# alexcoca/DistributedKernelShap

Hardware: AMD Instinct MI355X
Metric: explanations/sec (2560 inst, 100-sample background) (higher is better)
Workload: dtype fp32; 1 GPU; model=adult-logreg (12 groups, D=50, n_out=2, logit link), global_batch=2560, background=100, nsamples=default(2M+2048), parallelism=dp1, device=cuda

## Files before the change

distributedkernelshap_amd/ops/hip/bindings.cpp:

```cpp
#include <torch/extension.h>
#include <ATen/hip/HIPContext.h>
#include <c10/hip/HIPStream.h>

#include <cstdint>

extern "C" void launch_fill_random_masks(
    uint8_t* masks, int B, int S, int M, int ne, int n_random,
    const float* cdf, const int* sizes, int n_sizes, int num_paired,
    uint32_t seed, const int32_t* inst_ids, hipStream_t stream);

extern "C" int launch_fused_predict_linear(
    const uint8_t* masksU, const float* diff, const float* base, const float* wbg,
    float* ey, int B, int S, int M, int Mpad, int Npad, int n_out, int act,
    hipStream_t stream);

extern "C" void launch_synth_chunk(
    const uint8_t* masks, const float* x, const float* bg, const int* col_group,
    void* out, int out_bf16, int S, int M, int N, int D, int b_lo, int b_hi,
    int s_lo, int s_hi, hipStream_t stream);

extern "C" void launch_pack_masks(
    const uint8_t* masks, uint64_t* packed, int B, int S, int M,
    hipStream_t stream);

extern "C" int launch_fused_predict_bf16(
    const uint8_t* masksU, const uint16_t* diffB,
    const float* base, const float* wbg, float* ey, int B, int S, int M,
    int Npad, int n_out, int act, int split, hipStream_t stream);

extern "C" void launch_build_diff_f32(
    const float* xp, const float* bgp, const int64_t* vidx, float* out,
    int B, int G, int O, int N, int m, int Mpad, int Npad, hipStream_t stream);

extern "C" void launch_build_diff_bf16(
    const float* xp, const float* bgp, const int64_t* vidx, uint16_t* out,
    int B, int G, int O, int N, int m, int Npad, int split, hipStream_t stream);

extern "C" int launch_wls_solve(
    const uint8_t* masks, const uint64_t* packed, const float* kw,
    const float* ey_adj, const float* total, float* phi, int B, int S, int M,
    int n_out, hipStream_t stream);

extern "C" void launch_pack_masks_words(
    const uint8_t* masks, uint64_t* packed, int B, int S, int M, int W,
    hipStream_t stream);

extern "C" int launch_wls_gram(
    const uint64_t* packed, const float* kw, const float* ey_adj,
    const float* total, double* A64, double* rhs64, int B, int S, int M,
    int W, int n_out, hipStream_t stream);

extern "C" int launch_fused_predict_tiled(
    const uint8_t* masksU, const float* diff, const float* base,
    const float* wbg, float* partial, float* ey, int B, int S, int M,
    int Mpad, int Npad, int n_out, int act, hipStream_t stream);

extern "C" void launch_build_diff_bf16_tiled(
    const float* xp, const float* bgp, const int64_t* vidx, uint16_t* out,
    int B, int G, int O, int N, int m, int Mpad, int Npad, int split,
    hipStream_t stream);

extern "C" int launch_fused_predict_tiled_bf16(
    const uint8_t* masksU, const uint16_t* diffB, const float* base,
    const float* wbg, float* partial, float* ey, int B, int S, int M,
    int Mpad, int Npad, int n_out, int act, int split, hipStream_t stream);

extern "C" int launch_fill_masks_packed(
    uint64_t* packed, const uint64_t* enum_packed, int B, int S, int M, int ne,
    int n_random, const float* cdf, const int* sizes, int n_sizes,
    int num_paired, uint32_t seed, const int32_t* inst_ids, hipStream_t stream);

extern "C" int launch_linear_prepare(
    const float* X, const float* W, const float* bias,
    const int64_t* col_group, const int64_t* vidx, const float* bgp,
    const double* lfnull64, float* diff, float* total, int B, int D, int G,
    int N, int m, int Mpad, int Npad, int n_out, int act, int link,
    hipStream_t stream);

extern "C" int launch_fused_predict_linear_packed(
    const uint64_t* packed, const float* diff, const float* base,
    const float* wbg, const float* lfnull, float* ey, int B, int S, int Mpad,
    int Npad, int n_out, int act, int link, hipStream_t stream, int mma);

extern "C" int launch_wls_solve_packed(
    const uint64_t* packed, const float* kw, const float* ey_adj,
    const float* total, const int64_t* vidx, float* phi_full, int B, int S,
    int M, int n_out, int G, hipStream_t stream);

extern "C" int launch_varying_probe(
    const float* X, const float* bg_min, const float* bg_max,
    const float* tol_min, const float* tol_max, const int64_t* col_group,
    int64_t* keys, int64_t* probe, int B, int D, int G, hipStream_t stream);

extern "C" int launch_fused_predict_mlp(
    const uint8_t* masks, const void* xp1, const void* bgp1n,
    const float* base1, const void* const* hw, const float* const* hb,
    const int* H, int nhid, const void* wout, const float* bout,
    const float* wbg, float* ey, int B, int S, int M, int Mpad, int N,
    int n_out, int act, int hidden_act, int is_bf16, int nsplit,
    hipStream_t stream);

extern "C" int launch_fused_predict_trees(
    const uint8_t* masks, const int* vmap, const int64_t* dx, const int64_t* dbg,
    const uint8_t* child, const int* meta, const float* leaves,
    const int* grp_off, const int* grp_id, const int64_t* grp_mask,
    const float* base, const float* wbg, float* ey, float scale,
    int B, int S, int Mv, int N, int T, int G, int E, int L, int C,
    int max_internal, int n_out, int act, int leaf_mode, hipStream_t stream);

extern "C" int launch_fused_predict_trees_walk(
    const uint8_t* masks, const int* vmap, const float* x, const float* bg,
    const int* nodes, const int* roots, const float* leaves, const float* base,
    const float* wbg, float* ey, float scale,
    int B, int S, int Mv, int N, int D, int G, int T, int R, int L,
    int max_depth, int n_out, int act, int leaf_mode,
    const unsigned* cat_left, int C, hipStream_t stream);

extern "C" int launch_fused_predict_kernelmachine(
    const uint8_t* masks, const float* xp, const float* bgpn,
    const float* base, const float* alpha, const float* icpt,
    const float* wbg, float* ey, int B, int S, int M, int Mpad, int N,
    int Vpad, int n_out, int act, int kernel, float gamma, float coef0,
    int degree, hipStream_t stream);

namespace {

#define CHECK_DEV(t) TORCH_CHECK((t).is_cuda() && (t).is_contiguous(), #t " must be a contiguous device tensor")

hipStream_t current_stream() {
    return c10::hip::getCurrentHIPStream().stream();
}

void fill_random_masks(
    torch::Tensor masks, int64_t ne, int64_t n_random,
    torch::Tensor cdf, torch::Tensor sizes, int64_t num_paired, int64_t seed,
    torch::Tensor inst_ids) {
    CHECK_DEV(masks); CHECK_DEV(cdf); CHECK_DEV(sizes); CHECK_DEV(inst_ids);
    TORCH_CHECK(masks.dtype() == torch::kUInt8, "masks must be uint8");
    TORCH_CHECK(masks.dim() == 3, "masks must be (B,S,M)");
    TORCH_CHECK(inst_ids.dtype() == torch::kInt32, "inst_ids must be int32");
    int B = masks.size(0), S = masks.size(1), M = masks.size(2);
    TORCH_CHECK(inst_ids.size(0) == B, "inst_ids length");
    TORCH_CHECK(M <= 256, "fill_random_masks supports M <= 256");
    launch_fill_random_masks(
        masks.data_ptr<uint8_t>(), B, S, M, (int)ne, (int)n_random,
        cdf.data_ptr<float>(), sizes.data_ptr<int>(), (int)cdf.size(0),
        (int)num_paired, (uint32_t)seed, inst_ids.data_ptr<int32_t>(),
        current_stream());
}

void fused_predict_linear(
    torch::Tensor masks, torch::Tensor diff, torch::Tensor base,
    torch::Tensor wbg, torch::Tensor ey, int64_t act) {
    CHECK_DEV(masks); CHECK_DEV(diff); CHECK_DEV(base); CHECK_DEV(wbg); CHECK_DEV(ey);
    TORCH_CHECK(masks.dtype() == torch::kUInt8, "masks must be u8 (B,S,M)");
    int B = masks.size(0), S = masks.size(1), M = masks.size(2);
    int Mpad = diff.size(2), Npad = diff.size(3);
    int n_out = ey.size(2);
    int oimg = (act == 3) ? 1 : n_out;
    TORCH_CHECK(diff.size(1) == oimg, "diff image count vs act");
    TORCH_CHECK(M <= Mpad, "M vs Mpad");
    TORCH_CHECK(ey.size(0) == B && ey.size(1) == S, "ey shape");
    TORCH_CHECK(base.size(0) == oimg && base.size(1) == Npad, "base shape");
    TORCH_CHECK(wbg.size(0) == Npad, "wbg shape");
    int rc = launch_fused_predict_linear(
        masks.data_ptr<uint8_t>(), diff.data_ptr<float>(), base.data_ptr<float>(),
        wbg.data_ptr<float>(), ey.data_ptr<float>(), B, S, M, Mpad, Npad,
        n_out, (int)act, current_stream());
    TORCH_CHECK(rc == 0, "fused_predict_linear: unsupported shape (Mpad<=64, Npad%16==0, Npad<=128, n_out in {1,2,4})");
}

void synth_chunk(
    torch::Tensor masks, torch::Tensor x, torch::Tensor bg,
    torch::Tensor col_group, torch::Tensor out, int64_t b_lo, int64_t b_hi,
    int64_t s_lo, int64_t s_hi) {
    CHECK_DEV(masks); CHECK_DEV(x); CHECK_DEV(bg); CHECK_DEV(col_group); CHECK_DEV(out);
    int S = masks.size(1), M = masks.size(2);
    int N = bg.size(0), D = bg.size(1);
    TORCH_CHECK(out.size(0) == (b_hi - b_lo) * (s_hi - s_lo) * N && out.size(1) == D,
                "out shape");
    const bool bf16 = out.dtype() == torch::kBFloat16;
    TORCH_CHECK(bf16 || out.dtype() == torch::kFloat32,
                "out must be float32 or bfloat16");
    launch_synth_chunk(
        masks.data_ptr<uint8_t>(), x.data_ptr<float>(), bg.data_ptr<float>(),
        col_group.data_ptr<int>(),
        bf16 ? (void*)out.data_ptr<at::BFloat16>()
             : (void*)out.data_ptr<float>(),
        bf16 ? 1 : 0, S, M, N, D,
        (int)b_lo, (int)b_hi, (int)s_lo, (int)s_hi, current_stream());
}

void wls_solve(
    torch::Tensor masks, torch::Tensor kw, torch::Tensor ey_adj,
    torch::Tensor total, torch::Tensor phi,
    c10::optional<torch::Tensor> packed) {
    CHECK_DEV(masks); CHECK_DEV(kw); CHECK_DEV(ey_adj); CHECK_DEV(total); CHECK_DEV(phi);
    int B = masks.size(0), S = masks.size(1), M = masks.size(2);
    int n_out = ey_adj.size(2);
    TORCH_CHECK(phi.size(0) == B && phi.size(1) == M && phi.size(2) == n_out, "phi shape");
    const uint64_t* pk = nullptr;
    if (packed.has_value()) {
        CHECK_DEV(packed.value());
        TORCH_CHECK(packed->size(0) == B && packed->size(1) == S, "packed shape");
        pk = reinterpret_cast<const uint64_t*>(packed->data_ptr<int64_t>());
    }
    int rc = launch_wls_solve(
        masks.data_ptr<uint8_t>(), pk, kw.data_ptr<float>(), ey_adj.data_ptr<float>(),
        total.data_ptr<float>(), phi.data_ptr<float>(), B, S, M, n_out,
        current_stream());
    TORCH_CHECK(rc == 0, "wls_solve: unsupported shape (2<=M<=64, n_out<=8)");
}

void pack_masks(torch::Tensor masks, torch::Tensor packed) {
    CHECK_DEV(masks); CHECK_DEV(packed);
    TORCH_CHECK(masks.dtype() == torch::kUInt8, "masks must be u8");
    int B = masks.size(0), S = masks.size(1), M = masks.size(2);
    TORCH_CHECK(M <= 64, "pack_masks supports M <= 64");
    TORCH_CHECK(packed.size(0) == B && packed.size(1) == S, "packed shape");
    launch_pack_masks(
        masks.data_ptr<uint8_t>(),
        reinterpret_cast<uint64_t*>(packed.data_ptr<int64_t>()),
        B, S, M, current_stream());
}

#define CHECK_F32(t) TORCH_CHECK((t).dtype() == torch::kFloat32, #t " must be float32")
#define CHECK_I64(t) TORCH_CHECK((t).dtype() == torch::kInt64, #t " must be int64")

void fill_masks_packed(
    torch::Tensor packed, torch::Tensor enum_packed, int64_t n_random,
    torch::Tensor cdf, torch::Tensor sizes, int64_t num_paired, int64_t seed,
    torch::Tensor inst_ids, int64_t M) {
    CHECK_DEV(packed); CHECK_DEV(enum_packed); CHECK_DEV(cdf); CHECK_DEV(sizes);
    CHECK_DEV(inst_ids);
    CHECK_I64(packed); CHECK_I64(enum_packed); CHECK_F32(cdf);
    TORCH_CHECK(sizes.dtype() == torch::kInt32, "sizes must be int32");
    TORCH_CHECK(inst_ids.dtype() == torch::kInt32, "inst_ids must be int32");
    TORCH_CHECK(packed.dim() == 2 && enum_packed.dim() == 1,
                "packed must be (B,S), enum_packed (ne,)");
    int B = packed.size(0), S = packed.size(1), ne = enum_packed.size(0);
    TORCH_CHECK(inst_ids.dim() == 1 && inst_ids.size(0) == B, "inst_ids length");
    TORCH_CHECK(n_random >= 0 && ne + n_random == S, "ne + n_random must equal S");
    TORCH_CHECK(cdf.dim() == 1 && sizes.dim() == 1
                && cdf.size(0) == sizes.size(0), "cdf vs sizes");
    TORCH_CHECK(n_random == 0 || cdf.size(0) >= 1, "empty size table");
    int rc = launch_fill_masks_packed(
        reinterpret_cast<uint64_t*>(packed.data_ptr<int64_t>()),
        reinterpret_cast<const uint64_t*>(enum_packed.data_ptr<int64_t>()),
        B, S, (int)M, ne, (int)n_random, cdf.data_ptr<float>(),
        sizes.data_ptr<int>(), (int)cdf.size(0), (int)num_paired,
        (uint32_t)seed, inst_ids.data_ptr<int32_t>(), current_stream());
    TORCH_CHECK(rc == 0, "fill_masks_packed: unsupported shape (1<=M<=64)");
}

void linear_prepare(
    torch::Tensor X, torch::Tensor W, torch::Tensor bias,
    torch::Tensor col_group, torch::Tensor vidx, torch::Tensor bgp,
    torch::Tensor lfnull64, torch::Tensor diff, torch::Tensor total,
    int64_t act, int64_t link) {
    CHECK_DEV(X); CHECK_DEV(W); CHECK_DEV(bias); CHECK_DEV(col_group);
    CHECK_DEV(vidx); CHECK_DEV(bgp); CHECK_DEV(lfnull64); CHECK_DEV(diff);
    CHECK_DEV(total);
    CHECK_F32(X); CHECK_F32(W); CHECK_F32(bias); CHECK_F32(bgp); CHECK_F32(diff);
    CHECK_F32(total); CHECK_I64(col_group); CHECK_I64(vidx);
    TORCH_CHECK(lfnull64.dtype() == torch::kFloat64, "lfnull64 must be float64");
    TORCH_CHECK(X.dim() == 2 && W.dim() == 2 && bgp.dim() == 3 && diff.dim() == 4
                && total.dim() == 2 && vidx.dim() == 1, "operand ranks");
    int B = X.size(0), D = X.size(1), n_out = W.size(0);
    int N = bgp.size(0), G = bgp.size(1), OI = bgp.size(2), m = vidx.size(0);
    int Mpad = diff.size(2), Npad = diff.size(3);
    TORCH_CHECK(W.size(1) == D && bias.numel() == n_out
                && col_group.numel() == D && lfnull64.numel() == n_out,
                "W (n_out,D), b (n_out), col_group (D), lfnull64 (n_out)");
    TORCH_CHECK(OI == (act == 3 ? 1 : n_out), "background image count vs act");
    TORCH_CHECK(diff.size(0) == B && diff.size(1) == OI, "diff (B,OI,Mpad,Npad)");
    TORCH_CHECK(total.size(0) == B && total.size(1) == n_out, "total (B,n_out)");
    TORCH_CHECK(link == 0 || link == 1, "link must be 0 or 1");
    int rc = launch_linear_prepare(
        X.data_ptr<float>(), W.data_ptr<float>(), bias.data_ptr<float>(),
        col_group.data_ptr<int64_t>(), vidx.data_ptr<int64_t>(),
        bgp.data_ptr<float>(), lfnull64.data_ptr<double>(),
        diff.data_ptr<float>(), total.data_ptr<float>(), B, D, G, N, m, Mpad,
        Npad, n_out, (int)act, (int)link, current_stream());
    TORCH_CHECK(rc == 0, "linear_prepare: unsupported shape (m<=Mpad, m<=64, "
                         "N<=Npad, n_out<=8, act 3 needs n_out==2)");
}

void fused_predict_linear_packed(
    torch::Tensor packed, torch::Tensor diff, torch::Tensor base,
    torch::Tensor wbg, torch::Tensor ey, int64_t act, int64_t link,
    c10::optional<torch::Tensor> lfnull, int64_t mma) {
    CHECK_DEV(packed); CHECK_DEV(diff); CHECK_DEV(base); CHECK_DEV(wbg); CHECK_DEV(ey);
    CHECK_I64(packed); CHECK_F32(diff); CHECK_F32(base); CHECK_F32(wbg); CHECK_F32(ey);
    TORCH_CHECK(packed.dim() == 2 && diff.dim() == 4 && ey.dim() == 3
                && base.dim() == 2, "operand ranks");
    int B = packed.size(0), S = packed.size(1);
    int Mpad = diff.size(2), Npad = diff.size(3);
    int n_out = ey.size(2);
    int oimg = (act == 3) ? 1 : n_out;
    TORCH_CHECK(diff.size(0) == B && diff.size(1) == oimg, "diff (B,oimg,Mpad,Npad) vs act");
    TORCH_CHECK(ey.size(0) == B && ey.size(1) == S, "ey shape");
    TORCH_CHECK(base.size(0) == oimg && base.size(1) == Npad, "base shape");
    TORCH_CHECK(wbg.numel() == Npad, "wbg shape");
    const float* lf = nullptr;
    if (lfnull.has_value()) {
        CHECK_DEV(lfnull.value()); CHECK_F32(lfnull.value());
        TORCH_CHECK(lfnull->numel() == n_out, "lfnull must be (n_out,)");
        lf = lfnull->data_ptr<float>();
    }
    TORCH_CHECK(link == 0 || (link == 1 && lf != nullptr),
                "link must be 0, or 1 with lfnull given");
    TORCH_CHECK(mma >= -1 && mma <= 1,
                "mma must be -1 (auto), 0 (fp32 MFMA) or 1 (split bf16 MFMA)");
    int rc = launch_fused_predict_linear_packed(
        reinterpret_cast<const uint64_t*>(packed.data_ptr<int64_t>()),
        diff.data_ptr<float>(), base.data_ptr<float>(), wbg.data_ptr<float>(),
        lf, ey.data_ptr<float>(), B, S, Mpad, Npad, n_out, (int)act, (int)link,
        current_stream(), (int)mma);
    TORCH_CHECK(rc == 0, "fused_predict_linear_packed: unsupported shape "
                         "(Mpad%4==0, Mpad<=64, Npad%16==0, Npad<=128, n_out in "
                         "{1,2,4}, operand images within 64 KiB of LDS)");
}

void wls_solve_packed(
    torch::Tensor packed, torch::Tensor kw, torch::Tensor ey_adj,
    torch::Tensor total, torch::Tensor vidx, torch::Tensor phi_full) {
    CHECK_DEV(packed); CHECK_DEV(kw); CHECK_DEV(ey_adj); CHECK_DEV(total);
    CHECK_DEV(vidx); CHECK_DEV(phi_full);
    CHECK_I64(packed); CHECK_F32(kw); CHECK_F32(ey_adj); CHECK_F32(total);
    CHECK_I64(vidx); CHECK_F32(phi_full);
    TORCH_CHECK(packed.dim() == 2 && ey_adj.dim() == 3 && phi_full.dim() == 3
                && vidx.dim() == 1 && total.dim() == 2, "operand ranks");
    int B = packed.size(0), S = packed.size(1), M = vidx.size(0);
    int n_out = ey_adj.size(2), G = phi_full.size(1);
    TORCH_CHECK(kw.numel() == S, "kw must be (S,)");
    TORCH_CHECK(ey_adj.size(0) == B && ey_adj.size(1) == S, "ey_adj shape");
    TORCH_CHECK(total.size(0) == B && total.size(1) == n_out, "total shape");
    TORCH_CHECK(phi_full.size(0) == B && phi_full.size(2) == n_out, "phi_full shape");
    int rc = launch_wls_solve_packed(
        reinterpret_cast<const uint64_t*>(packed.data_ptr<int64_t>()),
        kw.data_ptr<float>(), ey_adj.data_ptr<float>(), total.data_ptr<float>(),
        vidx.data_ptr<int64_t>(), phi_full.data_ptr<float>(), B, S, M, n_out,
        G, current_stream());
    TORCH_CHECK(rc == 0, "wls_solve_packed: unsupported shape (2<=M<=G, "
                         "(M-1)+n_out<=16)");
}

void varying_probe(
    torch::Tensor X, torch::Tensor bg_min, torch::Tensor bg_max,
    torch::Tensor tol_min, torch::Tensor tol_max, torch::Tensor col_group,
    int64_t n_groups, torch::Tensor keys, torch::Tensor probe) {
    CHECK_DEV(X); CHECK_DEV(bg_min); CHECK_DEV(bg_max); CHECK_DEV(tol_min);
    CHECK_DEV(tol_max); CHECK_DEV(col_group); CHECK_DEV(keys); CHECK_DEV(probe);
    CHECK_F32(X); CHECK_F32(bg_min); CHECK_F32(bg_max); CHECK_F32(tol_min);
    CHECK_F32(tol_max); CHECK_I64(col_group); CHECK_I64(keys); CHECK_I64(probe);
    TORCH_CHECK(X.dim() == 2, "X must be (B,D)");
    const int64_t B = X.size(0), D = X.size(1);
    TORCH_CHECK(B >= 1 && D >= 1 && B <= 0x7fffffffLL && D <= 0x7fffffffLL,
                "X must be (B,D) with B, D >= 1");
    TORCH_CHECK(bg_min.numel() == D && bg_max.numel() == D
                && tol_min.numel() == D && tol_max.numel() == D
                && col_group.numel() == D,
                "bg_min, bg_max, tol_min, tol_max, col_group must be (D,)");
    TORCH_CHECK(keys.numel() == B, "keys must be (B,)");
    TORCH_CHECK(probe.numel() == 2, "probe must be (2,)");
    int rc = launch_varying_probe(
        X.data_ptr<float>(), bg_min.data_ptr<float>(), bg_max.data_ptr<float>(),
        tol_min.data_ptr<float>(), tol_max.data_ptr<float>(),
        col_group.data_ptr<int64_t>(), keys.data_ptr<int64_t>(),
        probe.data_ptr<int64_t>(), (int)B, (int)D, (int)n_groups,
        current_stream());
    TORCH_CHECK(rc == 0, "varying_probe: unsupported shape (1 <= n_groups <= 62)");
}

void fused_predict_bf16(
    torch::Tensor masks, torch::Tensor diffB, torch::Tensor base,
    torch::Tensor wbg, torch::Tensor ey, int64_t act) {
    CHECK_DEV(masks); CHECK_DEV(diffB); CHECK_DEV(base); CHECK_DEV(wbg); CHECK_DEV(ey);
    TORCH_CHECK(masks.dtype() == torch::kUInt8 && diffB.dtype() == torch::kBFloat16);
    int B = masks.size(0), S = masks.size(1), M = masks.size(2);
    int split = diffB.size(1), Npad = diffB.size(3);
    int n_out = ey.size(2);
    TORCH_CHECK(diffB.size(2) == ((act == 3) ? 1 : n_out), "diffB image count vs act");
    TORCH_CHECK(diffB.size(0) == B && diffB.size(4) == 40, "diffB (B,split,o,Npad,40)");
    TORCH_CHECK(ey.size(0) == B && ey.size(1) == S, "ey shape");
    int rc = launch_fused_predict_bf16(
        masks.data_ptr<uint8_t>(),
        reinterpret_cast<const uint16_t*>(diffB.data_ptr<at::BFloat16>()),
        base.data_ptr<float>(), wbg.data_ptr<float>(), ey.data_ptr<float>(),
        B, S, M, Npad, n_out, (int)act, split, current_stream());
    TORCH_CHECK(rc == 0, "fused_predict_bf16: unsupported shape (M<=32, Npad<=128, n_out in {1,2,4}, split in {1,2})");
}

void build_diff_f32(torch::Tensor xp, torch::Tensor bgp, torch::Tensor vidx,
                    torch::Tensor out) {
    CHECK_DEV(xp); CHECK_DEV(bgp); CHECK_DEV(vidx); CHECK_DEV(out);
    int B = xp.size(0), G = xp.size(1), O = xp.size(2);
    int N = bgp.size(0), m = vidx.size(0);
    int Mpad = out.size(2), Npad = out.size(3);
    TORCH_CHECK(out.size(0) == B && out.size(1) == O && m <= Mpad && N <= Npad);
    launch_build_diff_f32(
        xp.data_ptr<float>(), bgp.data_ptr<float>(), vidx.data_ptr<int64_t>(),
        out.data_ptr<float>(), B, G, O, N, m, Mpad, Npad, current_stream());
}

void build_diff_bf16(torch::Tensor xp, torch::Tensor bgp, torch::Tensor vidx,
                     torch::Tensor out) {
    CHECK_DEV(xp); CHECK_DEV(bgp); CHECK_DEV(vidx); CHECK_DEV(out);
    TORCH_CHECK(out.dtype() == torch::kBFloat16 && out.size(4) == 40);
    int B = xp.size(0), G = xp.size(1), O = xp.size(2);
    int N = bgp.size(0), m = vidx.size(0);
    int split = out.size(1), Npad = out.size(3);
    TORCH_CHECK(out.size(0) == B && out.size(2) == O && N <= Npad && m <= 32);
    launch_build_diff_bf16(
        xp.data_ptr<float>(), bgp.data_ptr<float>(), vidx.data_ptr<int64_t>(),
        reinterpret_cast<uint16_t*>(out.data_ptr<at::BFloat16>()), B, G, O, N,
        m, Npad, split, current_stream());
}

void pack_masks_words(torch::Tensor masks, torch::Tensor packed) {
    CHECK_DEV(masks); CHECK_DEV(packed);
    TORCH_CHECK(masks.dtype() == torch::kUInt8, "masks must be u8");
    TORCH_CHECK(packed.dim() == 3, "packed must be (B,S,W)");
    int B = masks.size(0), S = masks.size(1), M = masks.size(2);
    int W = packed.size(2);
    TORCH_CHECK(packed.size(0) == B && packed.size(1) == S, "packed shape");
    TORCH_CHECK(W * 64 >= M, "packed word count vs M");
    launch_pack_masks_words(
        masks.data_ptr<uint8_t>(),
        reinterpret_cast<uint64_t*>(packed.data_ptr<int64_t>()),
        B, S, M, W, current_stream());
}

void wls_gram(
    torch::Tensor packed, torch::Tensor kw, torch::Tensor ey_adj,
    torch::Tensor total, torch::Tensor A64, torch::Tensor rhs64) {
    CHECK_DEV(packed); CHECK_DEV(kw); CHECK_DEV(ey_adj); CHECK_DEV(total);
    CHECK_DEV(A64); CHECK_DEV(rhs64);
    TORCH_CHECK(packed.dim() == 3, "packed must be (B,S,W)");
    TORCH_CHECK(A64.dtype() == torch::kFloat64 && rhs64.dtype() == torch::kFloat64);
    int B = packed.size(0), S = packed.size(1), W = packed.size(2);
    int mm = A64.size(1), n_out = ey_adj.size(2);
    TORCH_CHECK(A64.size(0) == B && A64.size(2) == mm, "A64 shape");
    TORCH_CHECK(rhs64.size(0) == B && rhs64.size(1) == mm
                && rhs64.size(2) == n_out, "rhs64 shape");
    TORCH_CHECK(W * 64 >= mm + 1, "packed word count vs M");
    int rc = launch_wls_gram(
        reinterpret_cast<const uint64_t*>(packed.data_ptr<int64_t>()),
        kw.data_ptr<float>(), ey_adj.data_ptr<float>(),
        total.data_ptr<float>(), A64.data_ptr<double>(),
        rhs64.data_ptr<double>(), B, S, mm + 1, W, n_out, current_stream());
    TORCH_CHECK(rc == 0, "wls_gram: unsupported shape (M<=513, n_out<=8)");
}

void fused_predict_tiled(
    torch::Tensor masks, torch::Tensor diff, torch::Tensor base,
    torch::Tensor wbg, torch::Tensor partial, torch::Tensor ey, int64_t act) {
    CHECK_DEV(masks); CHECK_DEV(diff); CHECK_DEV(base); CHECK_DEV(wbg);
    CHECK_DEV(partial); CHECK_DEV(ey);
    TORCH_CHECK(masks.dtype() == torch::kUInt8, "masks must be u8 (B,S,M)");
    int B = masks.size(0), S = masks.size(1), M = masks.size(2);
    int Mpad = diff.size(2), Npad = diff.size(3);
    int n_out = ey.size(2);
    int oimg = (act == 3) ? 1 : n_out;
    int nacc = n_out;
    int n_ntiles = (Npad + 127) / 128;
    TORCH_CHECK(diff.size(1) == oimg, "diff image count vs act");
    TORCH_CHECK(M <= Mpad, "M vs Mpad");
    TORCH_CHECK(ey.size(0) == B && ey.size(1) == S, "ey shape");
    TORCH_CHECK(base.size(0) == oimg && base.size(1) == Npad, "base shape");
    TORCH_CHECK(wbg.size(0) == Npad, "wbg shape");
    TORCH_CHECK(partial.size(0) == B && partial.size(1) == n_ntiles
                && partial.size(2) == S && partial.size(3) == nacc,
                "partial shape (B, n_ntiles, S, nacc)");
    int rc = launch_fused_predict_tiled(
        masks.data_ptr<uint8_t>(), diff.data_ptr<float>(),
        base.data_ptr<float>(), wbg.data_ptr<float>(),
        partial.data_ptr<float>(), ey.data_ptr<float>(), B, S, M, Mpad,
        Npad, n_out, (int)act, current_stream());
    TORCH_CHECK(rc == 0, "fused_predict_tiled: unsupported shape "
                         "(Mpad%16==0, Npad%16==0, n_out in {1,2,4})");
}

void build_diff_bf16_tiled(torch::Tensor xp, torch::Tensor bgp,
                           torch::Tensor vidx, torch::Tensor out) {
    CHECK_DEV(xp); CHECK_DEV(bgp); CHECK_DEV(vidx); CHECK_DEV(out);
    TORCH_CHECK(out.dtype() == torch::kBFloat16 && out.dim() == 5,
                "out must be bf16 (B,split,O,Npad,Mpad)");
    int B = xp.size(0), G = xp.size(1), O = xp.size(2);
    int N = bgp.size(0), mcount = vidx.size(0);
    int split = out.size(1), Npad = out.size(3), Mpad = out.size(4);
    TORCH_CHECK(out.size(0) == B && out.size(2) == O && N <= Npad
                && mcount <= Mpad);
    launch_build_diff_bf16_tiled(
        xp.data_ptr<float>(), bgp.data_ptr<float>(), vidx.data_ptr<int64_t>(),
        reinterpret_cast<uint16_t*>(out.data_ptr<at::BFloat16>()), B, G, O, N,
        mcount, Mpad, Npad, split, current_stream());
}
// ... 186 lines not shown
    const int N = bg.size(0);
    TORCH_CHECK(nodes.dtype() == torch::kInt32 && nodes.dim() == 2
                && nodes.size(1) == 4, "nodes must be int32 (R,4)");
    TORCH_CHECK(roots.dtype() == torch::kInt32 && roots.dim() == 1,
                "roots must be int32 (T)");
    TORCH_CHECK(leaf_mode == 0 || leaf_mode == 1, "leaf_mode must be 0 or 1");
    TORCH_CHECK(leaves.dtype() == torch::kFloat32
                && (leaf_mode == 0 ? leaves.dim() == 1
                                   : (leaves.dim() == 2 && leaves.size(1) == n_out)),
                "leaves must be f32 (L) for scalar or (L,n_out) for vector leaves");
    TORCH_CHECK(base.dtype() == torch::kFloat32 && base.numel() == n_out,
                "base must be f32 (n_out)");
    TORCH_CHECK(wbg.dtype() == torch::kFloat32 && wbg.numel() == N,
                "wbg must be f32 (N)");
    TORCH_CHECK(max_depth >= 0 && max_depth <= 64, envelope);
    const unsigned* cat_ptr = nullptr;
    int64_t C = 0;
    if (cat_left.has_value()) {
        const torch::Tensor& cl = *cat_left;
        CHECK_DEV(cl);
        TORCH_CHECK(cl.dtype() == torch::kInt32 && cl.dim() == 2
                    && cl.size(1) == 8 && cl.size(0) >= 1,
                    "cat_left must be int32 (C,8) with C >= 1");
        TORCH_CHECK(cl.size(0) <= 0x7fffffffLL / 8, envelope);
        cat_ptr = reinterpret_cast<const unsigned*>(cl.data_ptr<int>());
        C = cl.size(0);
    }
    TORCH_CHECK(nodes.size(0) <= 0x7fffffffLL && leaves.size(0) <= 0x7fffffffLL
                && roots.size(0) <= 0x7fffffffLL && D <= 0x7fffffffLL
                && vmap.size(0) <= 0x7fffffffLL, envelope);
    int rc = launch_fused_predict_trees_walk(
        masks.data_ptr<uint8_t>(), vmap.data_ptr<int>(), x.data_ptr<float>(),
        bg.data_ptr<float>(), nodes.data_ptr<int>(), roots.data_ptr<int>(),
        leaves.data_ptr<float>(), base.data_ptr<float>(), wbg.data_ptr<float>(),
        ey.data_ptr<float>(), (float)scale, B, S, Mv, N, (int)D,
        (int)vmap.size(0), (int)roots.size(0), (int)nodes.size(0),
        (int)leaves.size(0), (int)max_depth, n_out, (int)act, (int)leaf_mode,
        cat_ptr, (int)C, current_stream());
    TORCH_CHECK(rc != -2, "fused_predict_trees_walk: LDS size attribute rejected");
    TORCH_CHECK(rc == 0, envelope);
}

void fused_predict_kernelmachine(
    torch::Tensor masks, torch::Tensor xp, torch::Tensor bgpn,
    torch::Tensor base, torch::Tensor alpha, torch::Tensor intercept,
    torch::Tensor wbg, torch::Tensor ey, int64_t kernel, double gamma,
    double coef0, int64_t degree, int64_t act) {
    static const char* envelope =
        "fused_predict_kernelmachine: outside the supported envelope (rbf or "
        "poly of degree 1-8, at most 2048 support vectors after padding to "
        "16, n_out <= 8, M <= Mpad <= 64 with Mpad a multiple of 16)";
    CHECK_DEV(masks); CHECK_DEV(xp); CHECK_DEV(bgpn); CHECK_DEV(base);
    CHECK_DEV(alpha); CHECK_DEV(intercept); CHECK_DEV(wbg); CHECK_DEV(ey);
    TORCH_CHECK(masks.dtype() == torch::kUInt8 && masks.dim() == 3,
                "masks must be u8 (B,S,M)");
    TORCH_CHECK(xp.dtype() == torch::kFloat32 && xp.dim() == 3,
                "xp must be f32 (B,Vpad,Mpad)");
    const int B = masks.size(0), S = masks.size(1), M = masks.size(2);
    const int Vpad = xp.size(1), Mpad = xp.size(2);
    TORCH_CHECK(xp.size(0) == B, "xp must be f32 (B,Vpad,Mpad)");
    TORCH_CHECK(bgpn.dtype() == torch::kFloat32 && bgpn.dim() == 3
                && bgpn.size(1) == Vpad && bgpn.size(2) == Mpad,
                "bgpn must be f32 (N,Vpad,Mpad)");
    const int N = bgpn.size(0);
    TORCH_CHECK(base.dtype() == torch::kFloat32 && base.dim() == 2
                && base.size(0) == N && base.size(1) == Vpad,
                "base must be f32 (N,Vpad)");
    TORCH_CHECK(alpha.dtype() == torch::kFloat32 && alpha.dim() == 2
                && alpha.size(0) == 16 && alpha.size(1) == Vpad,
                "alpha must be f32 (16,Vpad)");
    TORCH_CHECK(intercept.dtype() == torch::kFloat32 && intercept.numel() == 16,
                "intercept must be f32 (16)");
    TORCH_CHECK(wbg.dtype() == torch::kFloat32 && wbg.numel() == N,
                "wbg must be f32 (N)");
    TORCH_CHECK(ey.dtype() == torch::kFloat32 && ey.dim() == 3
                && ey.size(0) == B && ey.size(1) == S,
                "ey must be f32 (B,S,n_out)");
    const int n_out = ey.size(2);
    int rc = launch_fused_predict_kernelmachine(
        masks.data_ptr<uint8_t>(), xp.data_ptr<float>(), bgpn.data_ptr<float>(),
        base.data_ptr<float>(), alpha.data_ptr<float>(),
        intercept.data_ptr<float>(), wbg.data_ptr<float>(),
        ey.data_ptr<float>(), B, S, M, Mpad, N, Vpad, n_out, (int)act,
        (int)kernel, (float)gamma, (float)coef0, (int)degree, current_stream());
    TORCH_CHECK(rc == 0, envelope);
}

}

PYBIND11_MODULE(TORCH_EXTENSION_NAME, m) {
    m.def("fused_predict_kernelmachine", &fused_predict_kernelmachine,
          "fused kernel-machine predict (K4k): distance / dot product folded "
          "over varying groups, support vectors streamed in tiles of 16, "
          "kernel evaluation and the contraction with alpha on chip",
          pybind11::arg("masks"), pybind11::arg("xp"), pybind11::arg("bgpn"),
          pybind11::arg("base"), pybind11::arg("alpha"),
          pybind11::arg("intercept"), pybind11::arg("wbg"), pybind11::arg("ey"),
          pybind11::arg("kernel"), pybind11::arg("gamma"),
          pybind11::arg("coef0"), pybind11::arg("degree"), pybind11::arg("act"));
    m.def("fused_predict_trees", &fused_predict_trees,
          "fused tree-ensemble predict (K4t): per-tree node masks in LDS, "
          "bitwise select of packed x / background decisions, bit-register walk",
          pybind11::arg("masks"), pybind11::arg("vmap"), pybind11::arg("dx"),
          pybind11::arg("dbg"), pybind11::arg("child"), pybind11::arg("meta"),
          pybind11::arg("leaves"), pybind11::arg("grp_off"),
          pybind11::arg("grp_id"), pybind11::arg("grp_mask"),
          pybind11::arg("base"), pybind11::arg("scale"), pybind11::arg("wbg"),
          pybind11::arg("ey"), pybind11::arg("act"), pybind11::arg("leaf_mode"),
          pybind11::arg("max_internal"));
    m.def("fused_predict_trees_walk", &fused_predict_trees_walk,
          "fused deep-tree predict (K4w): 16-byte node records walked on the "
          "blended row, group bitset per sample, x row and background in LDS",
          pybind11::arg("masks"), pybind11::arg("vmap"), pybind11::arg("x"),
          pybind11::arg("bg"), pybind11::arg("nodes"), pybind11::arg("roots"),
          pybind11::arg("leaves"), pybind11::arg("base"),
          pybind11::arg("scale"), pybind11::arg("wbg"), pybind11::arg("ey"),
          pybind11::arg("act"), pybind11::arg("leaf_mode"),
          pybind11::arg("max_depth"),
          pybind11::arg("cat_left") = pybind11::none());
    m.def("fused_predict_mlp", &fused_predict_mlp,
          "fused MLP predict (K4m): first layer folded over varying groups, "
          "hidden activations in LDS, f32 or bf16 MFMA by operand dtype",
          pybind11::arg("masks"), pybind11::arg("xp1"), pybind11::arg("bgp1n"),
          pybind11::arg("base1"), pybind11::arg("hidden_w"),
          pybind11::arg("hidden_b"), pybind11::arg("wout"),
          pybind11::arg("bout"), pybind11::arg("wbg"), pybind11::arg("ey"),
          pybind11::arg("act"), pybind11::arg("hidden_act") = 0);
    m.def("fill_masks_packed", &fill_masks_packed,
          "Philox coalition sampling straight into packed u64 words (K2p): "
          "bit-identical to the enumerated-row copy, fill_random_masks and "
          "pack_masks in sequence, M <= 64",
          pybind11::arg("packed"), pybind11::arg("enum_packed"),
          pybind11::arg("n_random"), pybind11::arg("cdf"),
          pybind11::arg("sizes"), pybind11::arg("num_paired"),
          pybind11::arg("seed"), pybind11::arg("inst_ids"), pybind11::arg("M"));
    m.def("linear_prepare", &linear_prepare,
          "per-call operand prep for the packed linear pipeline (K0p): diff "
          "image in the build_diff_f32 layout plus the fp64-evaluated totals",
          pybind11::arg("X"), pybind11::arg("W"), pybind11::arg("b"),
          pybind11::arg("col_group"), pybind11::arg("vidx"),
          pybind11::arg("bgp"), pybind11::arg("lfnull64"),
          pybind11::arg("diff"), pybind11::arg("total"), pybind11::arg("act"),
          pybind11::arg("link"));
    m.def("fused_predict_linear_packed", &fused_predict_linear_packed,
          "MFMA fused predict from packed mask words with the link fused into "
          "the epilogue (K3p); mma: -1 auto, 0 fp32 MFMA, 1 split-operand bf16 "
          "MFMA (Mpad <= 12, act 1/3; other shapes take the fp32 MFMA path)",
          pybind11::arg("packed"), pybind11::arg("diff"), pybind11::arg("base"),
          pybind11::arg("wbg"), pybind11::arg("ey"), pybind11::arg("act"),
          pybind11::arg("link") = 0, pybind11::arg("lfnull") = pybind11::none(),
          pybind11::arg("mma") = -1);
    m.def("wls_solve_packed", &wls_solve_packed,
          "MFMA WLS solve with (S,) kernel weights, scattered into "
          "phi_full (B,G,n_out) through vidx (K7p)",
          pybind11::arg("packed"), pybind11::arg("kw"), pybind11::arg("ey_adj"),
          pybind11::arg("total"), pybind11::arg("vidx"),
          pybind11::arg("phi_full"));
    m.def("varying_probe", &varying_probe,
          "varying-pattern probe (K1p): per-instance group bit keys and "
          "[all(keys == keys[0]), keys[0]] in two launches, no host sync",
          pybind11::arg("X"), pybind11::arg("bg_min"), pybind11::arg("bg_max"),
          pybind11::arg("tol_min"), pybind11::arg("tol_max"),
          pybind11::arg("col_group"), pybind11::arg("n_groups"),
          pybind11::arg("keys"), pybind11::arg("probe"));
    m.def("fill_random_masks", &fill_random_masks,
          "Philox coalition sampling (K2)");
    m.def("fused_predict_linear", &fused_predict_linear,
          "MFMA fused mask@diff GEMM + activation + background reduce (K3-K6)");
    m.def("build_diff_f32", &build_diff_f32,
          "diff image in the f32 fused-kernel layout");
    m.def("build_diff_bf16", &build_diff_bf16,
          "hi(+lo) diff images in the bf16 fused-kernel layout");
    m.def("pack_masks", &pack_masks,
          "masks u8 -> packed u64 bits (for the MFMA WLS Gram build)");
    m.def("fused_predict_bf16", &fused_predict_bf16,
          "bf16 matrix-core fused predict (single or hi+lo split), A-operand "
          "converted in-register from the raw u8 masks");
    m.def("synth_chunk", &synth_chunk,
          "masked-background perturbation synthesis tile (K3')");
    m.def("wls_solve", &wls_solve,
          "batched constrained WLS Shapley solve (K7)",
          pybind11::arg("masks"), pybind11::arg("kw"), pybind11::arg("ey_adj"),
          pybind11::arg("total"), pybind11::arg("phi"),
          pybind11::arg("packed") = pybind11::none());
    m.def("pack_masks_words", &pack_masks_words,
          "masks u8 -> (B,S,W) packed u64 words (wide-M Gram build)");
    m.def("wls_gram", &wls_gram,
          "tiled MFMA Gram+rhs build (fp64 via chunked promotion) for the "
          "stress WLS shapes, M up to 513");
    m.def("fused_predict_tiled", &fused_predict_tiled,
          "tiled MFMA fused predict for Mpad>64 / Npad>128 (LDS-streamed "
          "diff chunks, per-column-tile partials + deterministic reduce)");
    m.def("build_diff_bf16_tiled", &build_diff_bf16_tiled,
          "hi(+lo) k-contiguous diff image for the bf16 tiled predict");
    m.def("fused_predict_tiled_bf16", &fused_predict_tiled_bf16,
          "bf16 matrix-core tiled fused predict (v_mfma_f32_16x16x32_bf16 "
          "per 32-deep k block; hi+lo split for fp32-grade)");
}
```

distributedkernelshap_amd/ops/hip/kshap_kernels.hip:

```cpp

#include <hip/hip_runtime.h>
#include <cstdint>
#include <type_traits>

#include "split_bf16.h"

#define WAVE 64


struct Philox {
    uint32_t ctr[4];
    uint32_t key[2];
    uint32_t buf[4];
    int idx;

    __device__ void init(uint32_t k0, uint32_t k1, uint32_t c0, uint32_t c1) {
        key[0] = k0; key[1] = k1;
        ctr[0] = c0; ctr[1] = c1; ctr[2] = 0; ctr[3] = 0;
        idx = 4;
    }
    __device__ static void round_(uint32_t c[4], const uint32_t k[2]) {
        const uint32_t M0 = 0xD2511F53u, M1 = 0xCD9E8D57u;
        uint64_t p0 = (uint64_t)M0 * c[0];
        uint64_t p1 = (uint64_t)M1 * c[2];
// ... 2355 lines not shown
                           : arow == 2 ? partial[o][2] : partial[o][3];
            }
            if (link == 1) {
#pragma unroll
                for (int o = 0; o < NOUT; ++o) {
                    const float p = fminf(fmaxf(out[o], 1e-7f), 0.9999999f);
                    out[o] = 0.69314718055994530942f
                        * (__builtin_amdgcn_logf(p) - __builtin_amdgcn_logf(1.0f - p));
                }
            }
            if (lfnull != nullptr) {
#pragma unroll
                for (int o = 0; o < NOUT; ++o) out[o] -= lfnull[o];
            }
            float* dst = ey + ((size_t)b * S + ss) * NOUT;
            if constexpr (NOUT == 2) {
                *(float2*)dst = make_float2(out[0], out[1]);
            } else if constexpr (NOUT == 4) {
                *(float4*)dst = make_float4(out[0], out[1], out[2], out[3]);
            } else {
                dst[0] = out[0];
            }
        }
    }
}

template <int NOUT, int ACT, int NT>
static int launch_fpp_ks(
    const uint64_t* packed, const float* diff, const float* base,
    const float* wbg, const float* lfnull, float* ey, int B, int S, int Mpad,
    int link, int mma, hipStream_t stream)
{
    const int n_stiles = (S + S_TILE - 1) / S_TILE;
    dim3 grid(B * n_stiles), block(256);
    constexpr int NPAD = NT * 16;
    constexpr int NSTRIDE = NPAD + ((16 - (NPAD & 31)) & 31);
    constexpr int OIMG = (ACT == 3) ? 1 : NOUT;
    size_t lds = (size_t)(OIMG * Mpad * NSTRIDE + OIMG * NPAD + NPAD) * 4;
    if (lds > 64 * 1024) return -1;
#define KSHAP_FPP(KSV, MMAV) \
    fused_predict_linear_packed_kernel<NOUT, ACT, NT, KSV, MMAV> \
        <<<grid, block, lds, stream>>>(packed, diff, base, wbg, lfnull, ey, \
                                       B, S, Mpad, link)
    if constexpr (ACT == 1 || ACT == 3) {
        const size_t lds_split = (size_t)OIMG * NT * 64 * 32 + (size_t)NPAD * 4;
        if (mma != 0 && Mpad <= 12 && lds_split <= 64 * 1024) {
            lds = lds_split;
            switch (Mpad / 4) {
                case 1: KSHAP_FPP(1, 1); return 0;
                case 2: KSHAP_FPP(2, 1); return 0;
                case 3: KSHAP_FPP(3, 1); return 0;
                default: break;
            }
        }
        switch (Mpad / 4) {
            case 1: KSHAP_FPP(1, 0); return 0;
            case 2: KSHAP_FPP(2, 0); return 0;
            case 3: KSHAP_FPP(3, 0); return 0;
            case 4: KSHAP_FPP(4, 0); return 0;
            default: break;
        }
    }
    KSHAP_FPP(0, 0);
#undef KSHAP_FPP
    return 0;
}

template <int NOUT, int ACT>
static int launch_fpp_nt(
    const uint64_t* packed, const float* diff, const float* base,
    const float* wbg, const float* lfnull, float* ey, int B, int S, int Mpad,
    int Npad, int link, int mma, hipStream_t stream)
{
#define KSHAP_FPP_NT(NTV) \
    case NTV: \
        return launch_fpp_ks<NOUT, ACT, NTV>(packed, diff, base, wbg, lfnull, \
                                             ey, B, S, Mpad, link, mma, stream);
    switch (Npad / 16) {
        KSHAP_FPP_NT(1) KSHAP_FPP_NT(2) KSHAP_FPP_NT(3) KSHAP_FPP_NT(4)
        KSHAP_FPP_NT(5) KSHAP_FPP_NT(6) KSHAP_FPP_NT(7) KSHAP_FPP_NT(8)
    }
#undef KSHAP_FPP_NT
    return -1;
}

template <int NOUT>
static int launch_fpp_act(
    const uint64_t* packed, const float* diff, const float* base,
    const float* wbg, const float* lfnull, float* ey, int B, int S, int Mpad,
    int Npad, int act, int link, int mma, hipStream_t stream)
{
    switch (act) {
        case 0:
            return launch_fpp_nt<NOUT, 0>(packed, diff, base, wbg, lfnull, ey, B, S, Mpad, Npad, link, mma, stream);
        case 1:
            return launch_fpp_nt<NOUT, 1>(packed, diff, base, wbg, lfnull, ey, B, S, Mpad, Npad, link, mma, stream);
        case 2:
            return launch_fpp_nt<NOUT, 2>(packed, diff, base, wbg, lfnull, ey, B, S, Mpad, Npad, link, mma, stream);
        case 3:
            if constexpr (NOUT == 2)
                return launch_fpp_nt<NOUT, 3>(packed, diff, base, wbg, lfnull, ey, B, S, Mpad, Npad, link, mma, stream);
            return -1;
        default:
            return -1;
    }
}

extern "C" int launch_fused_predict_linear_packed(
    const uint64_t* packed, const float* diff, const float* base,
    const float* wbg, const float* lfnull, float* ey, int B, int S, int Mpad,
    int Npad, int n_out, int act, int link, hipStream_t stream, int mma)
{
    if (Mpad < 4 || Mpad > MAX_MPAD || Mpad % 4 != 0 || Npad % 16 != 0
            || Npad < 16 || Npad / 16 > 8 || mma < -1 || mma > 1)
        return -1;
    if (link != 0 && (link != 1 || lfnull == nullptr)) return -1;
    if (B <= 0 || S <= 0) return 0;
    switch (n_out) {
        case 1: return launch_fpp_act<1>(packed, diff, base, wbg, lfnull, ey, B, S, Mpad, Npad, act, link, mma, stream);
        case 2: return launch_fpp_act<2>(packed, diff, base, wbg, lfnull, ey, B, S, Mpad, Npad, act, link, mma, stream);
        case 4: return launch_fpp_act<4>(packed, diff, base, wbg, lfnull, ey, B, S, Mpad, Npad, act, link, mma, stream);
        default: return -1;
    }
}

template <int J>
__device__ __forceinline__ float dpp_row_bcast(float v) {
    return __builtin_bit_cast(float, __builtin_amdgcn_update_dpp(
        0, __builtin_bit_cast(int, v), 0x150 + J, 0xF, 0xF, true));
}
template <int J>
__device__ __forceinline__ uint32_t dpp_row_bcast_u(uint32_t v) {
    return (uint32_t)__builtin_amdgcn_update_dpp(0, (int)v, 0x150 + J, 0xF, 0xF, true);
}

template <int I, int N, class F>
__device__ __forceinline__ void static_for(F&& f) {
    if constexpr (I < N) {
        f(std::integral_constant<int, I>{});
        static_for<I + 1, N>(f);
    }
}

#define WLSP_MAXM 15

template <int NOUT>
struct WlsSample {
    uint32_t bits;
    float w;
    float e[NOUT];
    bool ok;
};

template <int NOUT>
__global__ __launch_bounds__(64)
void wls_solve_packed_kernel(
    const uint64_t* __restrict__ packed,
    const float* __restrict__ kw,
    const float* __restrict__ ey_adj,
    const float* __restrict__ total,
    const int64_t* __restrict__ vidx,
    float* __restrict__ phi_full,
    int B, int S, int M, int n_out, int G)
{
    const int b = blockIdx.x;
    if (b >= B) return;
    const int lane = threadIdx.x;
    const int arow = lane & 15;
    const int akk = lane >> 4;
    const int mm = M - 1;

    __shared__ float As[16][17];
    __shared__ float phi_s[16][NOUT];
    __shared__ int g_s[16];

    float tot[NOUT];
#pragma unroll
    for (int o = 0; o < NOUT; ++o)
        tot[o] = o < n_out ? total[(size_t)b * n_out + o] : 0.0f;
    if (lane < M) g_s[lane] = (int)vidx[lane];

    const uint64_t* pbase = packed + (size_t)b * S;
    const float* eyb = ey_adj + (size_t)b * S * n_out;
    const int slot = 4 * arow + akk;
    const bool is_a = arow < mm;
    const int osel = arow - mm;

    auto load = [&](int base) __attribute__((always_inline)) {
        WlsSample<NOUT> s;
        s.ok = base + slot < S;
        const int idx = min(base + slot, S - 1);
        s.bits = (uint32_t)pbase[idx];
        s.w = kw[idx];
#pragma unroll
        for (int o = 0; o < NOUT; ++o)
            s.e[o] = eyb[(size_t)idx * n_out + min(o, n_out - 1)];
        return s;
    };

    auto gram_block = [&](f32x4& acc, const WlsSample<NOUT>& raw, int rem) __attribute__((always_inline)) {
        WlsSample<NOUT> s;
        s.bits = raw.ok ? raw.bits : 0u;
        s.w = raw.ok ? raw.w : 0.0f;
        const float ml = (float)((s.bits >> mm) & 1u);
        float wey[NOUT];
#pragma unroll
        for (int o = 0; o < NOUT; ++o)
            wey[o] = o < n_out ? s.w * (raw.e[o] - ml * tot[o]) : 0.0f;
        static_for<0, 16>([&](auto jc) __attribute__((always_inline)) {
            constexpr int j = decltype(jc)::value;
            if (4 * j < rem) {
                const uint32_t bb = dpp_row_bcast_u<j>(s.bits);
                const float ww = dpp_row_bcast<j>(s.w);
                float es = 0.0f;
#pragma unroll
                for (int o = 0; o < NOUT; ++o) {
                    const float t = dpp_row_bcast<j>(wey[o]);
                    es = (osel == o) ? t : es;
                }
                const float d = (float)((int)((bb >> arow) & 1u)
                                        - (int)((bb >> mm) & 1u));
                const float a = is_a ? d : 0.0f;
                const float bv = is_a ? ww * d : es;
                acc = __builtin_amdgcn_mfma_f32_16x16x4f32(a, bv, acc, 0, 0, 0);
            }
        });
    };

    f32x4 acc[4];
#pragma unroll
    for (int w = 0; w < 4; ++w) acc[w] = (f32x4){0, 0, 0, 0};

    WlsSample<NOUT> cur = load(0);
    for (int c0 = 0; c0 < S; c0 += WLS_CHUNK) {
        static_for<0, 4>([&](auto wc) __attribute__((always_inline)) {
            constexpr int w = decltype(wc)::value;
            const int base = c0 + w * 64;
            if (base < S) {
                const WlsSample<NOUT> nxt = load(base + 64);
                gram_block(acc[w], cur, S - base);
                cur = nxt;
            }
        });
    }
#pragma unroll
    for (int r = 0; r < 4; ++r)
        As[akk * 4 + r][arow] = ((acc[0][r] + acc[1][r]) + acc[2][r]) + acc[3][r];
    __syncthreads();

    float L[WLSP_MAXM];
#pragma unroll
    for (int c = 0; c < WLSP_MAXM; ++c) {
        const float v = As[arow][c];
        L[c] = (arow < mm && c < mm) ? v : (arow == c ? 1.0f : 0.0f);
    }
    static_for<0, WLSP_MAXM>([&](auto kc) __attribute__((always_inline)) {
        constexpr int k = decltype(kc)::value;
        const float d = sqrtf(fmaxf(dpp_row_bcast<k>(L[k]), 1e-20f));
        const float inv = 1.0f / d;
        const float lk = L[k] * inv;
        L[k] = (arow == k) ? d : lk;
        static_for<k + 1, WLSP_MAXM>([&](auto cc) __attribute__((always_inline)) {
            constexpr int c = decltype(cc)::value;
            L[c] = fmaf(-lk, dpp_row_bcast<c>(lk), L[c]);
        });
    });

#pragma unroll 1
    for (int o0 = 0; o0 < NOUT; o0 += 4) {
        const int o = o0 + akk;
        const bool live = o < n_out;
        const float r_own = (live && arow < mm) ? As[arow][mm + (live ? o : 0)] : 0.0f;
        float y[WLSP_MAXM], wv[WLSP_MAXM];
        static_for<0, WLSP_MAXM>([&](auto ic) __attribute__((always_inline)) {
            constexpr int i = decltype(ic)::value;
            float v = dpp_row_bcast<i>(r_own);
            static_for<0, i>([&](auto tc) __attribute__((always_inline)) {
                constexpr int t = decltype(tc)::value;
                v = fmaf(-dpp_row_bcast<i>(L[t]), y[t], v);
            });
            y[i] = v / dpp_row_bcast<i>(L[i]);
        });
        static_for<0, WLSP_MAXM>([&](auto ic) __attribute__((always_inline)) {
            constexpr int i = WLSP_MAXM - 1 - decltype(ic)::value;
            float v = y[i];
            static_for<i + 1, WLSP_MAXM>([&](auto tc) __attribute__((always_inline)) {
                constexpr int t = decltype(tc)::value;
                v = fmaf(-dpp_row_bcast<t>(L[i]), wv[t], v);
            });
            wv[i] = v / dpp_row_bcast<i>(L[i]);
        });
        float sumw = 0.0f;
#pragma unroll
        for (int i = 0; i < WLSP_MAXM; ++i) sumw += wv[i];
        if (live) {
            float mine = 0.0f;
#pragma unroll
            for (int i = 0; i < WLSP_MAXM; ++i) mine = (arow == i) ? wv[i] : mine;
            float to = 0.0f;
#pragma unroll
            for (int oo = 0; oo < NOUT; ++oo) to = (o == oo) ? tot[oo] : to;
            if (arow < mm) phi_s[arow][o] = mine;
            if (arow == mm) phi_s[mm][o] = to - sumw;
        }
    }
    __syncthreads();
    float* prow = phi_full + (size_t)b * G * n_out;
    for (int idx = lane; idx < G * n_out; idx += 64) {
        const int g = idx / n_out, o = idx % n_out;
        float v = 0.0f;
        for (int k = 0; k < M; ++k)
            if (g_s[k] == g) v = phi_s[k][o];
        prow[idx] = v;
    }
}

extern "C" int launch_wls_solve_packed(
    const uint64_t* packed, const float* kw, const float* ey_adj,
    const float* total, const int64_t* vidx, float* phi_full, int B, int S,
    int M, int n_out, int G, hipStream_t stream)
{
    if (M < 2 || M > G || n_out < 1 || n_out > WLS_MAX_NOUT
            || (M - 1) + n_out > 16)
        return -1;
    if (B <= 0) return 0;
#define KSHAP_WLSP(NO) \
    wls_solve_packed_kernel<NO><<<dim3(B), dim3(64), 0, stream>>>( \
        packed, kw, ey_adj, total, vidx, phi_full, B, S, M, n_out, G)
    if (n_out == 1) KSHAP_WLSP(1);
    else if (n_out == 2) KSHAP_WLSP(2);
    else if (n_out <= 4) KSHAP_WLSP(4);
    else KSHAP_WLSP(8);
#undef KSHAP_WLSP
    return 0;
}


__global__ __launch_bounds__(256)
void varying_keys_kernel(
    const float* __restrict__ X,
    const float* __restrict__ bg_min,
    const float* __restrict__ bg_max,
    const float* __restrict__ tol_min,
    const float* __restrict__ tol_max,
    const int64_t* __restrict__ col_group,
    int64_t* __restrict__ keys,
    int B, int D)
{
    const int lane = threadIdx.x & (WAVE - 1);
    const int b = blockIdx.x * (blockDim.x / WAVE) + (threadIdx.x >> 6);
    if (b >= B) return;
    const float* xr = X + (size_t)b * D;
    uint64_t bits = 0ull;
    for (int j = lane; j < D; j += WAVE) {
        const float x = xr[j];
        const bool cmin = fabsf(__fsub_rn(bg_min[j], x)) <= tol_min[j];
        const bool cmax = fabsf(__fsub_rn(bg_max[j], x)) <= tol_max[j];
        const int64_t g = col_group[j];
        if (!(cmin && cmax) && g >= 0 && g < 64) bits |= 1ull << g;
    }
    uint32_t lo = (uint32_t)bits, hi = (uint32_t)(bits >> 32);
#pragma unroll
    for (int off = 1; off < WAVE; off <<= 1) {
        lo |= (uint32_t)__shfl_xor((int)lo, off, WAVE);
        hi |= (uint32_t)__shfl_xor((int)hi, off, WAVE);
    }
    if (lane == 0) keys[b] = (int64_t)(((uint64_t)hi << 32) | lo);
}

__global__ __launch_bounds__(1024)
void varying_probe_reduce_kernel(
    const int64_t* __restrict__ keys,
    int64_t* __restrict__ probe,
    int B)
{
    const int64_t k0 = keys[0];
    int differs = 0;
    for (int i = threadIdx.x; i < B; i += blockDim.x)
        differs |= (keys[i] != k0);
    differs = __syncthreads_or(differs);
    if (threadIdx.x == 0) {
        probe[0] = differs ? 0 : 1;
        probe[1] = k0;
    }
}

extern "C" int launch_varying_probe(
    const float* X, const float* bg_min, const float* bg_max,
    const float* tol_min, const float* tol_max, const int64_t* col_group,
    int64_t* keys, int64_t* probe, int B, int D, int G, hipStream_t stream)
{
    if (B < 1 || D < 1 || G < 1 || G > 62) return -1;
    const int wpb = 256 / WAVE;
    varying_keys_kernel<<<dim3((B + wpb - 1) / wpb), dim3(256), 0, stream>>>(
        X, bg_min, bg_max, tol_min, tol_max, col_group, keys, B, D);
    varying_probe_reduce_kernel<<<dim3(1), dim3(1024), 0, stream>>>(
        keys, probe, B);
    return 0;
}
```

Baseline: 6.448 million explanations/s.

## Split WLS Gram accumulation across up to four waves per instance

The packed WLS solve kernel can now run with 1, 2 or 4 waves per instance block. The four Gram accumulator streams are divided among the waves, then combined through shared memory before wave 0 does the Cholesky solve. An auto heuristic based on B and S picks 4 waves when the batch is small relative to device capacity. The goal is to expose more parallelism in the Gram phase and cut per-instance latency. The cost is an extra LDS reduction and a block barrier, and the other waves sit idle during the solve phase.

```diff
diff --git a/distributedkernelshap_amd/ops/hip/bindings.cpp b/distributedkernelshap_amd/ops/hip/bindings.cpp
--- a/distributedkernelshap_amd/ops/hip/bindings.cpp
+++ b/distributedkernelshap_amd/ops/hip/bindings.cpp
@@ -85,7 +85,7 @@
 extern "C" int launch_wls_solve_packed(
     const uint64_t* packed, const float* kw, const float* ey_adj,
     const float* total, const int64_t* vidx, float* phi_full, int B, int S,
-    int M, int n_out, int G, hipStream_t stream);
+    int M, int n_out, int G, hipStream_t stream, int waves);
 
 extern "C" int launch_varying_probe(
     const float* X, const float* bg_min, const float* bg_max,
@@ -324,7 +324,8 @@
 
 void wls_solve_packed(
     torch::Tensor packed, torch::Tensor kw, torch::Tensor ey_adj,
-    torch::Tensor total, torch::Tensor vidx, torch::Tensor phi_full) {
+    torch::Tensor total, torch::Tensor vidx, torch::Tensor phi_full,
+    int64_t waves) {
     CHECK_DEV(packed); CHECK_DEV(kw); CHECK_DEV(ey_adj); CHECK_DEV(total);
     CHECK_DEV(vidx); CHECK_DEV(phi_full);
     CHECK_I64(packed); CHECK_F32(kw); CHECK_F32(ey_adj); CHECK_F32(total);
@@ -341,9 +342,9 @@
         reinterpret_cast<const uint64_t*>(packed.data_ptr<int64_t>()),
         kw.data_ptr<float>(), ey_adj.data_ptr<float>(), total.data_ptr<float>(),
         vidx.data_ptr<int64_t>(), phi_full.data_ptr<float>(), B, S, M, n_out,
-        G, current_stream());
+        G, current_stream(), (int)waves);
     TORCH_CHECK(rc == 0, "wls_solve_packed: unsupported shape (2<=M<=G, "
-                         "(M-1)+n_out<=16)");
+                         "(M-1)+n_out<=16, waves in {0 (auto), 1, 2, 4})");
 }
 
 void varying_probe(
@@ -836,10 +837,11 @@
           pybind11::arg("mma") = -1);
     m.def("wls_solve_packed", &wls_solve_packed,
           "MFMA WLS solve with (S,) kernel weights, scattered into "
-          "phi_full (B,G,n_out) through vidx (K7p)",
+          "phi_full (B,G,n_out) through vidx (K7p); waves per instance in the "
+          "Gram phase: 0 auto, or 1, 2, 4 (every choice gives the same bits)",
           pybind11::arg("packed"), pybind11::arg("kw"), pybind11::arg("ey_adj"),
           pybind11::arg("total"), pybind11::arg("vidx"),
-          pybind11::arg("phi_full"));
+          pybind11::arg("phi_full"), pybind11::arg("waves") = 0);
     m.def("varying_probe", &varying_probe,
           "varying-pattern probe (K1p): per-instance group bit keys and "
           "[all(keys == keys[0]), keys[0]] in two launches, no host sync",
diff --git a/distributedkernelshap_amd/ops/hip/kshap_kernels.hip b/distributedkernelshap_amd/ops/hip/kshap_kernels.hip
--- a/distributedkernelshap_amd/ops/hip/kshap_kernels.hip
+++ b/distributedkernelshap_amd/ops/hip/kshap_kernels.hip
@@ -2531,8 +2531,8 @@
     bool ok;
 };
 
-template <int NOUT>
-__global__ __launch_bounds__(64)
+template <int NOUT, int NW>
+__global__ __launch_bounds__(64 * NW)
 void wls_solve_packed_kernel(
     const uint64_t* __restrict__ packed,
     const float* __restrict__ kw,
@@ -2542,9 +2542,12 @@
     float* __restrict__ phi_full,
     int B, int S, int M, int n_out, int G)
 {
+    static_assert(NW == 1 || NW == 2 || NW == 4, "waves per instance");
+    constexpr int NA = 4 / NW;
     const int b = blockIdx.x;
     if (b >= B) return;
-    const int lane = threadIdx.x;
+    const int lane = threadIdx.x & (WAVE - 1);
+    const int wv = NW > 1 ? (int)(threadIdx.x >> 6) : 0;
     const int arow = lane & 15;
     const int akk = lane >> 4;
     const int mm = M - 1;
@@ -2552,12 +2555,13 @@
     __shared__ float As[16][17];
     __shared__ float phi_s[16][NOUT];
     __shared__ int g_s[16];
+    __shared__ f32x4 acc_s[NW > 1 ? 4 : 1][WAVE];
 
     float tot[NOUT];
 #pragma unroll
     for (int o = 0; o < NOUT; ++o)
         tot[o] = o < n_out ? total[(size_t)b * n_out + o] : 0.0f;
-    if (lane < M) g_s[lane] = (int)vidx[lane];
+    if ((int)threadIdx.x < M) g_s[threadIdx.x] = (int)vidx[threadIdx.x];
 
     const uint64_t* pbase = packed + (size_t)b * S;
     const float* eyb = ey_adj + (size_t)b * S * n_out;
@@ -2610,17 +2614,25 @@
 #pragma unroll
     for (int w = 0; w < 4; ++w) acc[w] = (f32x4){0, 0, 0, 0};
 
-    WlsSample<NOUT> cur = load(0);
+    WlsSample<NOUT> cur = load(wv * 64);
     for (int c0 = 0; c0 < S; c0 += WLS_CHUNK) {
-        static_for<0, 4>([&](auto wc) __attribute__((always_inline)) {
-            constexpr int w = decltype(wc)::value;
-            const int base = c0 + w * 64;
+        static_for<0, NA>([&](auto ic) __attribute__((always_inline)) {
+            constexpr int i = decltype(ic)::value;
+            const int base = c0 + (wv + i * NW) * 64;
             if (base < S) {
-                const WlsSample<NOUT> nxt = load(base + 64);
-                gram_block(acc[w], cur, S - base);
+                const WlsSample<NOUT> nxt = load(base + 64 * NW);
+                gram_block(acc[i], cur, S - base);
                 cur = nxt;
             }
         });
+    }
+    if constexpr (NW > 1) {
+#pragma unroll
+        for (int i = 0; i < NA; ++i) acc_s[wv + i * NW][lane] = acc[i];
+        __syncthreads();
+        if (wv != 0) return;
+#pragma unroll
+        for (int w = 0; w < 4; ++w) acc[w] = acc_s[w][lane];
     }
 #pragma unroll
     for (int r = 0; r < 4; ++r)
@@ -2694,24 +2706,50 @@
     }
 }
 
+template <int NOUT>
+static int launch_wlsp_waves(
+    const uint64_t* packed, const float* kw, const float* ey_adj,
+    const float* total, const int64_t* vidx, float* phi_full, int B, int S,
+    int M, int n_out, int G, int waves, hipStream_t stream)
+{
+#define KSHAP_WLSP(NWV) \
+    wls_solve_packed_kernel<NOUT, NWV><<<dim3(B), dim3(64 * NWV), 0, stream>>>( \
+        packed, kw, ey_adj, total, vidx, phi_full, B, S, M, n_out, G)
+    switch (waves) {
+        case 1: KSHAP_WLSP(1); return 0;
+        case 2: KSHAP_WLSP(2); return 0;
+        case 4: KSHAP_WLSP(4); return 0;
+        default: return -1;
+    }
+#undef KSHAP_WLSP
+}
+
+static int wlsp_auto_waves(int B, int S)
+{
+    if (S <= 64) return 1;
+    const long cost1 = 90 + 220L * ((B + 1023) / 1024);
+    const long cost4 = 75 + 62L * ((B + 255) / 256);
+    return cost4 < cost1 ? 4 : 1;
+}
+
 extern "C" int launch_wls_solve_packed(
     const uint64_t* packed, const float* kw, const float* ey_adj,
     const float* total, const int64_t* vidx, float* phi_full, int B, int S,
-    int M, int n_out, int G, hipStream_t stream)
+    int M, int n_out, int G, hipStream_t stream, int waves)
 {
     if (M < 2 || M > G || n_out < 1 || n_out > WLS_MAX_NOUT
-            || (M - 1) + n_out > 16)
+            || (M - 1) + n_out > 16
+            || (waves != 0 && waves != 1 && waves != 2 && waves != 4))
         return -1;
     if (B <= 0) return 0;
-#define KSHAP_WLSP(NO) \
-    wls_solve_packed_kernel<NO><<<dim3(B), dim3(64), 0, stream>>>( \
-        packed, kw, ey_adj, total, vidx, phi_full, B, S, M, n_out, G)
-    if (n_out == 1) KSHAP_WLSP(1);
-    else if (n_out == 2) KSHAP_WLSP(2);
-    else if (n_out <= 4) KSHAP_WLSP(4);
-    else KSHAP_WLSP(8);
-#undef KSHAP_WLSP
-    return 0;
+    if (waves == 0) waves = wlsp_auto_waves(B, S);
+    if (n_out == 1)
+        return launch_wlsp_waves<1>(packed, kw, ey_adj, total, vidx, phi_full, B, S, M, n_out, G, waves, stream);
+    if (n_out == 2)
+        return launch_wlsp_waves<2>(packed, kw, ey_adj, total, vidx, phi_full, B, S, M, n_out, G, waves, stream);
+    if (n_out <= 4)
+        return launch_wlsp_waves<4>(packed, kw, ey_adj, total, vidx, phi_full, B, S, M, n_out, G, waves, stream);
+    return launch_wlsp_waves<8>(packed, kw, ey_adj, total, vidx, phi_full, B, S, M, n_out, G, waves, stream);
 }
 
 
```

Result: slower. 6.227 million explanations/s (-3.4%).
